# probabilists/zuko

Hardware: AMD Instinct MI355X
Metric: log_prob samples/sec, NSF d=64 K=8 bins=8 batch=2^20 (higher is better)
Workload: dtype f32; 1 GPU; NSF(features=64, context=0, transforms=8, bins=8, hidden=[256]*3) log_prob, batch=2^20 per GPU, x~N(0,1), seed-0 init; batch_per_gpu=1048576, global_batch=1048576, parallelism=batch-sharded x1, one RCCL all-reduce of the scalar NLL

## Files before the change

zuko_amd/csrc/fused_ar_half_impl.h:

```cpp
#pragma once
#include "fused_ar_split_impl.h"

#ifndef ARH_LOOK
#define ARH_LOOK 1
#endif
#ifndef ARH_RELU_INT
#define ARH_RELU_INT 0
#endif
#ifndef ARH_EPI_PINNED
#define ARH_EPI_PINNED 1
#endif
#ifndef ARH_DESCALE_PK
#define ARH_DESCALE_PK 1
#endif
#ifndef ARH_PREFETCH
#define ARH_PREFETCH 1
#endif
#ifndef ARH_BLOCK_ASM
#define ARH_BLOCK_ASM 1
#endif
#ifndef ARH_EPI_TILE
#define ARH_EPI_TILE 1
#endif

namespace zk {

typedef _Float16 f16x8 __attribute__((ext_vector_type(8)));

struct ArhB {
  f16x8 h, l;
};

__device__ __forceinline__ void arh_scale(float& amax, float& s, float& inv_s) {
  amax = fmaxf(amax, __shfl_xor(amax, 16, 64));
  amax = fmaxf(amax, __shfl_xor(amax, 32, 64));
  int e = __builtin_amdgcn_frexp_expf(amax);
  int ea = 15 - e;
  ea = ea > 90 ? 90 : (ea < -90 ? -90 : ea);
  s = __builtin_amdgcn_ldexpf(1.0f, ea);
  inv_s = __builtin_amdgcn_ldexpf(1.0f, -ea);
}

#define ARH_AMAX_OVERFLOW (65520.f * 0x1p90f)

typedef unsigned arh_u32x4 __attribute__((ext_vector_type(4)));
typedef float arh_f32x2 __attribute__((ext_vector_type(2)));

__device__ __forceinline__ void arh_split(const f32x4& lo, const f32x4& hi, float s, ArhB& b) {
  if (ARX_ABL == 6) {
    b.h = __builtin_bit_cast(f16x8, lo); b.l = __builtin_bit_cast(f16x8, hi);
    return;
  }
#if ARH_EPI_PINNED
  const float nz = -0.f;
  unsigned h0, h1, h2, h3, l0, l1, l2, l3;
#define ARH_SPLIT_H(OP, H, V) "v_fma_mix" OP "_f16 %[" H "], %[" V "], %[s], %[nz]\n\t"
#define ARH_SPLIT_L(OP, SEL, L, H, V) "v_fma_mix" OP "_f16 %[" L "], %[" V "], %[s], -%[" H "] op_sel:[0,0," SEL "] op_sel_hi:[0,0,1]\n\t"
// ... 4 lines not shown
      : [h0] "=&v"(h0), [h1] "=&v"(h1), [h2] "=&v"(h2), [h3] "=&v"(h3), [l0] "=&v"(l0), [l1] "=&v"(l1), [l2] "=&v"(l2), [l3] "=&v"(l3)
      : [v0] "v"(lo[0]), [v1] "v"(lo[1]), [v2] "v"(lo[2]), [v3] "v"(lo[3]), [v4] "v"(hi[0]), [v5] "v"(hi[1]), [v6] "v"(hi[2]), [v7] "v"(hi[3]), [s] "v"(s), [nz] "s"(nz));
#undef ARH_SPLIT_H
#undef ARH_SPLIT_L
  b.h = __builtin_bit_cast(f16x8, arh_u32x4{h0, h1, h2, h3}); b.l = __builtin_bit_cast(f16x8, arh_u32x4{l0, l1, l2, l3});
  return;
#endif
#pragma unroll
  for (int e = 0; e < 8; ++e) {
    const float v = (e < 4 ? lo[e] : hi[e - 4]) * s;
    const _Float16 h = (_Float16)v;
    const float r = v - (float)h;
    b.h[e] = h;
    b.l[e] = (_Float16)r;
  }
}

#define ARH_MFMA(A, B, C) C = __builtin_amdgcn_mfma_f32_16x16x32_f16(__builtin_bit_cast(f16x8, A), B, C, 0, 0, 0)
__device__ __forceinline__ void arh_block(const f32x4 (&a)[2], const ArhB& b, f32x4& c) {
  if (ARX_ABL == 2) {
    asm volatile("" ::"v"(a[0]), "v"(a[1]));
    return;
  }
  ARH_MFMA(a[1], b.h, c);
  ARH_MFMA(a[0], b.l, c);
  ARH_MFMA(a[0], b.h, c);
}

__device__ __forceinline__ void arh_touch(f32x4& v) { asm volatile("" : "+v"(v)); }
template <int N> __device__ __forceinline__ void arh_settle(f32x4& a0, f32x4& a1) { asm volatile("s_waitcnt lgkmcnt(%2)" : "+v"(a0), "+v"(a1) : "n"(N)); }
template <int N> __device__ __forceinline__ void arh_settle(f32x4& a0, f32x4& a1, f32x4& a2) { asm volatile("s_waitcnt lgkmcnt(%3)" : "+v"(a0), "+v"(a1), "+v"(a2) : "n"(N)); }

constexpr bool ARH_BLK = ARH_BLOCK_ASM && ARX_ABL != 2;
#define ARH_BLK_ASM(C0, COUT, POST, BSOUT)                                                                  \
  asm volatile("v_mfma_f32_16x16x32_f16 %[c], %[al], %[bh], " C0 "\n\t"                                     \
               "v_mfma_f32_16x16x32_f16 %[c], %[ah], %[bl], %[c]\n\t"                                       \
               "v_mfma_f32_16x16x32_f16 %[c], %[ah], %[bh], %[c]" POST                                      \
               : [c] COUT(c) ARH_BLK_BS##BSOUT                                                              \
               : [ah] "v"(a[0]), [al] "v"(a[1]), [bh] "v"(b.h), [bl] "v"(b.l))
#define ARH_BLK_BS0
#define ARH_BLK_BS1 , "+v"(bs)
template <int N, bool FIRST, bool PAD, bool TILE> __device__ __forceinline__ void arh_wait_block(f32x4 (&a)[2], const ArhB& b, f32x4& c, f32x4& bs) {
  static_assert(N >= 0 && N < 16, "lgkmcnt is a four-bit field");
  if constexpr (PAD) asm volatile("s_nop 0");
  __builtin_amdgcn_s_waitcnt(0xC07F | (N << 8));
  if (ARX_FENCE) __builtin_amdgcn_sched_barrier(0);
  if constexpr (FIRST && TILE) ARH_BLK_ASM("0", "=&v", "\n\ts_nop 11", 1);
  else if constexpr (FIRST) ARH_BLK_ASM("0", "=&v", "", 0);
  else if constexpr (TILE) ARH_BLK_ASM("%[c]", "+v", "\n\ts_nop 11", 1);
  else ARH_BLK_ASM("%[c]", "+v", "", 0);
  if (ARX_FENCE) __builtin_amdgcn_sched_barrier(0);
}
#undef ARH_BLK_ASM
#undef ARH_BLK_BS0
#undef ARH_BLK_BS1
template <int NT> __device__ __forceinline__ void arh_acc_ready(f32x4 (&acc)[NT]) {
  asm volatile("s_nop 11" : "+v"(acc[NT - 1]));
#pragma unroll
  for (int t = 0; t + 1 < NT; ++t) arh_touch(acc[t]);
}

__device__ __forceinline__ void arh_relu_max(f32x4& o, float (&pm)[4], int t) {
#pragma unroll
  for (int r = 0; r < 4; r += 2)
    asm("v_max_f32 %0, 0, %0\n\tv_max_f32 %1, 0, %1\n\tv_max3_f32 %2, %2, %0, %1" : "+v"(o[r]), "+v"(o[r + 1]), "+v"(pm[(2 * t + r / 2) % 4]));
}
__device__ __forceinline__ float arh_join_max(const float (&pm)[4]) {
  float amax;
  asm("v_max_f32 %0, %1, %2\n\tv_max3_f32 %0, %0, %3, %4" : "=&v"(amax) : "v"(pm[0]), "v"(pm[1]), "v"(pm[2]), "v"(pm[3]));
  return amax;
}

template <int WAVES, int CH, int NR> struct ArhRing : ArRingS<WAVES, CH, NR> {
  typedef ArRingS<WAVES, CH, NR> B;
  template <int XV> __device__ __forceinline__ void advance_x() {
    asm volatile("s_waitcnt vmcnt(%0) lgkmcnt(0)" ::"n"((NR - 2) * B::PER + XV) : "memory");
    if (ARX_ABL != 4) __builtin_amdgcn_s_barrier();
    asm volatile("" ::: "memory");
    this->issue();
    this->slot = (this->slot + 1 == NR) ? 0 : this->slot + 1;
    this->cur_off = this->lds_off + (unsigned)(this->slot * CH * AR_TF * 4 + this->lane * 16);
  }
  template <int S, int XV = 0> __device__ __forceinline__ f32x4 read() {
    if constexpr (XV != 0 && S % CH == 0) {
      advance_x<XV>();
      f32x4 v;
      if (ARX_ABL == 5) {
        asm volatile("v_mov_b32 %0, %1" : "=v"(v[0]) : "v"(this->cur_off));
// ... 73 lines not shown
      wait<XV, DRAIN>();
    }
    if (ARX_ABL != 4) __builtin_amdgcn_s_barrier();
    asm volatile("" ::: "memory");
    issue();
    asm volatile("" ::: "memory");
  }
  template <int S, int XV = 0> __device__ __forceinline__ f32x4 read() {
    static_assert(S >= 0 && S < IMAGES, "stream position");
    if constexpr (S % CH == 0) {
      read_off = (read_off + CHB == NR * CHB) ? 0 : read_off + CHB;
      cur_off = lane_off + read_off;
    }
    f32x4 v;
    if (ARX_ABL == 5) {
      asm volatile("v_mov_b32 %0, %1" : "=v"(v[0]) : "v"(cur_off));
      v[1] = v[2] = v[3] = v[0];
    } else {
      asm volatile("ds_read_b128 %0, %1 offset:%2" : "=v"(v) : "v"(cur_off), "n"((S % CH) * AR_TF * 4));
    }
    if constexpr (S == trigger(S / CH)) boundary<XV, (S % CH != BPOS + 1)>();
    if constexpr (FLOW && NCH >= 2) {
      if constexpr (S == trigger(NCH - 2)) bias_request();
    }
    return v;
  }
};

template <class S, int L, bool ALT> constexpr int arh_ip(int s) {
  if constexpr (ALT) return S::B_IP_ALT[s];
  else return ArxPat<S>::ip(L, s);
}
template <class S> constexpr bool ARH_EPI = S::ACT == 1 && ARH_EPI_PINNED && ARH_EPI_TILE;
template <class S, int L, class Ring, bool ALT = false> __device__ __forceinline__ void arh_hidden(Ring& ring, const float* bias_q, const ArhB (&in)[S::TMAX / 2], f32x4 (&out)[S::TMAX], float d, float (&pm)[4]) {
  typedef ArxPat<S> P;
  constexpr int NB = S::NB[L], BASE = S::BASE[L], HTL = S::HT[L];
  ars_for<HTL>([&](auto t_) ARS_ALWAYS_INLINE {
    constexpr int t = t_;
    if constexpr (!P::tile_has_blocks(L, t)) {
      out[t] = *reinterpret_cast<const f32x4*>(bias_q + t * 16);
      if constexpr (ARH_EPI<S>) arh_relu_max(out[t], pm, t);
    }
  });
  if constexpr (NB > 0) {
    constexpr int LOOK = ARH_LOOK < NB ? ARH_LOOK : NB;
    f32x4 a[LOOK + 1][2];
    f32x4 bs;
    f32x4 acc;
    const unsigned bias_addr = arx_lds_addr(bias_q);
    ars_for<LOOK>([&](auto b_) ARS_ALWAYS_INLINE {
      constexpr int b = b_;
      ars_for<2>([&](auto p) ARS_ALWAYS_INLINE { a[b][p] = ring.template read<BASE + 2 * b + decltype(p)::value>(); });
    });
    ars_for<NB>([&](auto s_) ARS_ALWAYS_INLINE {
      constexpr int s = s_, ot = P::ot(L, s), cur = s % (LOOK + 1);
      constexpr int ip = arh_ip<S, L, ALT>(s);
      constexpr bool first_of_tile = (s == 0 || P::ot(L, s - 1) != ot), last_of_tile = (s + 1 == NB || P::ot(L, s + 1) != ot);
      if constexpr (first_of_tile && !ARH_BLK) acc = f32x4{0.f, 0.f, 0.f, 0.f};
      if constexpr (last_of_tile) bs = arx_lds_raw<ot * 64>(bias_addr);
      if constexpr (s + LOOK < NB) {
        constexpr int nx = (s + LOOK) % (LOOK + 1);
        ars_for<2>([&](auto p) ARS_ALWAYS_INLINE { a[nx][p] = ring.template read<BASE + 2 * (s + LOOK) + decltype(p)::value>(); });
      }
      constexpr int ahead = (s + LOOK < NB ? LOOK : NB - 1 - s);
      if constexpr (ARH_BLK) {
        arh_wait_block<(last_of_tile ? (s + LOOK < NB ? 2 : 0) : 2 * ahead), first_of_tile, s == 0, last_of_tile>(a[cur], in[ip], acc, bs);
      } else {
        if constexpr (last_of_tile) arh_settle<(s + LOOK < NB ? 2 : 0)>(a[cur][0], a[cur][1], bs);
        else arh_settle<2 * ahead>(a[cur][0], a[cur][1]);
        if (ARX_FENCE) __builtin_amdgcn_sched_barrier(0);
        arh_block(a[cur], in[ip], acc);
        if (ARX_FENCE) __builtin_amdgcn_sched_barrier(0);
      }
      if constexpr (last_of_tile) {
        if (ARH_DESCALE_PK) {
#pragma unroll
          for (int r = 0; r < 4; r += 2) {
            const arh_f32x2 o = __builtin_elementwise_fma(arh_f32x2{acc[r], acc[r + 1]}, arh_f32x2{d, d}, arh_f32x2{bs[r], bs[r + 1]});
            out[ot][r] = o[0]; out[ot][r + 1] = o[1];
          }
        } else {
#pragma unroll
          for (int r = 0; r < 4; ++r) out[ot][r] = __builtin_fmaf(acc[r], d, bs[r]);
        }
        if constexpr (ARH_EPI<S>) arh_relu_max(out[ot], pm, ot);
      }
    });
  }
}

template <class S, int L, class Ring, bool HAS_ALT = false> __device__ __forceinline__ void arh_hidden_stack(Ring& ring, const float* bias_lds, int q, ArhB (&in)[S::TMAX / 2], f32x4 (&out)[S::TMAX], const float* wd,
                                                                                                         float& inv_s, float& poison, bool alt = false) {
  if constexpr (L < S::NH) {
    float pm[4] = {0.f, 0.f, 0.f, 0.f};
    if constexpr (HAS_ALT && L == 0) {
      static_assert(S::BASE[0] == 0, "B_IP_ALT lists the first layer's blocks");
      if (alt) arh_hidden<S, L, Ring, true>(ring, bias_lds + L * S::BIAS_STRIDE + 4 * q, in, out, wd[L] * inv_s, pm);
      else arh_hidden<S, L, Ring>(ring, bias_lds + L * S::BIAS_STRIDE + 4 * q, in, out, wd[L] * inv_s, pm);
    } else {
      arh_hidden<S, L, Ring>(ring, bias_lds + L * S::BIAS_STRIDE + 4 * q, in, out, wd[L] * inv_s, pm);
    }
    constexpr int HTL = S::HT[L];
    float amax = 0.f;
    if constexpr (S::ACT == 1 && ARH_EPI_PINNED) {
      if constexpr (!ARH_EPI_TILE) {
#pragma unroll
        for (int t = 0; t < HTL; ++t) arh_relu_max(out[t], pm, t);
      }
      amax = arh_join_max(pm);
    } else if constexpr (S::ACT == 1) {
#pragma unroll
      for (int t = 0; t < HTL; ++t)
#pragma unroll
        for (int r = 0; r < 4; ++r) {
          if (ARH_RELU_INT) out[t][r] = __builtin_bit_cast(float, max(__builtin_bit_cast(int, out[t][r]), 0));
          else out[t][r] = out[t][r] < 0.f ? 0.f : out[t][r];
          amax = fmaxf(amax, out[t][r]);
        }
    } else {
      ar_activate<S::ACT, HTL>(out, out);
#pragma unroll
      for (int t = 0; t < HTL; ++t)
#pragma unroll
        for (int r = 0; r < 4; ++r) amax = fmaxf(amax, fabsf(out[t][r]));
    }
    float s;
    arh_scale(amax, s, inv_s);
    if constexpr (S::ACT == 1 && ARH_EPI_PINNED) {
      if (!(amax < ARH_AMAX_OVERFLOW)) poison = __builtin_nanf("");
    }
    const f32x4 zero = {0.f, 0.f, 0.f, 0.f};
#pragma unroll
    for (int p = 0; p < (HTL + 1) / 2; ++p) arh_split(out[2 * p], 2 * p + 1 < HTL ? out[2 * p + 1] : zero, s, in[p]);
    arh_hidden_stack<S, L + 1, Ring, HAS_ALT>(ring, bias_lds, q, in, out, wd, inv_s, poison, alt);
  }
}

template <typename Uni> __device__ __forceinline__ void arh_flow_epilogue(float (&p)[4 * Uni::NT], const ArArgs& a, const int (&fid)[Uni::FPL], const float (&xin)[Uni::FPL], float poison, float* xr,
                                                                          const float* base, int D, bool term, float& lacc) {
  constexpr int FPL = Uni::FPL, TOTAL = Uni::TOTAL;
#pragma unroll
  for (int fi = 0; fi < FPL; ++fi) Uni::template poison<false>(p, fi * TOTAL, poison);
  auto ld = [&](int i) { return p[i]; };
#pragma unroll
  for (int fi = 0; fi < FPL; ++fi) {
    const int f = fid[fi];
    if (f >= 0) {
      float yv, lj;
      Uni::fwd(ld, fi * TOTAL, a, xin[fi], yv, lj);
      lacc += lj;
      if (term) {
        const float df = yv - base[f];
        lacc += __builtin_fmaf(-(df * df), base[D + f], base[2 * D + f]);
      } else {
        xr[f] = yv;
      }
    }
  }
}

template <class S, typename Uni, bool DIAG, bool TERM, bool FLOW, class Ring, class XReq, class Fids>
__device__ __forceinline__ void arh_pass(const ArArgs& a, Ring& ring, XReq& x_request, f32x4 (&xnext)[S::NIT], float* bias_lds, const Fids& fids, float* xr, const float* base, const ArLane& ln,
                                         int64_t tile, const float* wd, bool first, bool last, bool term, float& total, bool alt = false) {
  constexpr bool RING4 = S::NR == 4;
  static_assert(!FLOW || (RING4 && S::XLDS && S::DIN == S::D && !DIAG && !TERM), "flow pass: four-slot ring, rows in LDS, no context columns");
  constexpr int NT = Uni::NT, FPL = Uni::FPL, WAVES = S::WAVES;
  constexpr int NG = S::NG;
// ... 21 lines not shown
    for (int it = 0; it < S::NIT; ++it) {
      f32x4 v = {0.f, 0.f, 0.f, 0.f};
      if constexpr (FLOW) {
        if ((it + 1) * 16 <= S::DIN || it * 16 + 4 * q < S::DIN) v = *reinterpret_cast<const f32x4*>(xr + it * 16 + 4 * q);
      } else if (ARH_PREFETCH) {
        if ((it + 1) * 16 <= S::DIN || it * 16 + 4 * q < S::DIN) v = xnext[it];
      } else {
        if ((it + 1) * 16 <= S::DIN || it * 16 + 4 * q < S::DIN) v = *reinterpret_cast<const f32x4*>(xrow + it * 16 + 4 * q);
      }
      xin[it] = v;
    }
    xin[S::NIT] = f32x4{0.f, 0.f, 0.f, 0.f};
    poison = ar_poison_of<S::NIT>(xin);
    float amax = 0.f;
#pragma unroll
    for (int it = 0; it < S::NIT; ++it)
#pragma unroll
      for (int r = 0; r < 4; ++r) amax = fmaxf(amax, fabsf(xin[it][r]));
    if constexpr (XLDS && !FLOW) ar_rows_in<S::D>(xr, q, xin);
    float s;
    arh_scale(amax, s, inv_s);
    if constexpr (S::ACT == 1 && ARH_EPI_PINNED) {
      if (!(amax < ARH_AMAX_OVERFLOW)) poison = __builtin_nanf("");
    }
#pragma unroll
    for (int p = 0; p < (S::NIT + 1) / 2; ++p) arh_split(xin[2 * p], xin[2 * p + 1], s, in[p]);
  }

  float ladj_in = 0.f;
  if constexpr (!FLOW) {
    if (ARH_PREFETCH && a.ladj && a.accumulate && live && q == 0) ladj_in = a.ladj[n];
  }

  if constexpr (FLOW) arh_hidden_stack<S, 0, Ring, S::FLOW_ALT>(ring, bias_lds, q, in, out, wd, inv_s, poison, alt);
  else arh_hidden_stack<S, 0, Ring>(ring, bias_lds, q, in, out, wd, inv_s, poison);

  const float dl = wd[S::NH] * inv_s;
  float lacc = 0.f;
  constexpr int NBL = NSTEP * NT;
  constexpr int LOOKL = ARH_LOOK < NBL ? ARH_LOOK : NBL;
  f32x4 w[LOOKL + 1][2];
  constexpr int XPOS = []() constexpr {
    if constexpr (!ARH_PREFETCH) return -1;
    else if constexpr (RING4) return Ring::first_trigger_from(S::LAST_BASE);
    else return (S::LAST_BASE + S::CH - 1) / S::CH * S::CH;
  }();
  if constexpr (FLOW) {
    asm volatile("" ::: "memory");
    if (last) {
      x_request(tile + gridDim.x < a.n_tiles ? tile + gridDim.x : tile, xnext);
    } else {
#pragma unroll
      for (int it = 0; it < S::NIT; ++it) asm("" : "=v"(xnext[it]));
    }
    ring.rows_in_flight = last;
    asm volatile("" ::: "memory");
  } else if (ARH_PREFETCH) {
    asm volatile("" ::: "memory");
    x_request(tile + gridDim.x < a.n_tiles ? tile + gridDim.x : tile, xnext);
    asm volatile("" ::: "memory");
  }
#define ARH_READ_LAST(POS) ring.template read<(POS), ((POS) == XPOS ? S::NIT : 0)>()
  ars_for<LOOKL>([&](auto b_) ARS_ALWAYS_INLINE {
    constexpr int b = b_;
    ars_for<2>([&](auto p) ARS_ALWAYS_INLINE { w[b][p] = ARH_READ_LAST(S::LAST_BASE + 2 * b + decltype(p)::value); });
  });
  ars_for<NG>([&](auto g_) ARS_ALWAYS_INLINE {
    constexpr int g = g_, ST0 = S::GOFF[g], GN = S::GOFF[g + 1] - S::GOFF[g];
    int fid[FPL];
    float xin[FPL];
    fids.template fetch<XLDS>(g, xr, xrow, fid, xin);
    float bv[3 * FPL];
    if constexpr (TERM && !FLOW) fids.fetch_base(fid, base, S::D, bv);
    f32x4 acc[NT], bs[NT];
    if constexpr (GN == 0) {
      const float* bg = bias_last + (g * NT) * 16 + 4 * q;
      ars_for<NT>([&](auto t) ARS_ALWAYS_INLINE { bs[t] = *reinterpret_cast<const f32x4*>(bg + t * 16); });
    }
    if constexpr (GN == 0 || !ARH_BLK) ars_for<NT>([&](auto t) ARS_ALWAYS_INLINE { acc[t] = f32x4{0.f, 0.f, 0.f, 0.f}; });
    ars_for<GN>([&](auto i_) ARS_ALWAYS_INLINE {
      constexpr int st = ST0 + decltype(i_)::value, ip = S::G_IP[st];
      ars_for<NT>([&](auto t_) ARS_ALWAYS_INLINE {
        constexpr int t = t_, blk = st * NT + t, cur = blk % (LOOKL + 1);
        constexpr bool last_of_group = (decltype(i_)::value == GN - 1 && t == NT - 1);
        if constexpr (last_of_group) {
          ars_for<NT>([&](auto u) ARS_ALWAYS_INLINE { bs[u] = arx_lds_raw<(g * NT + decltype(u)::value) * 64>(bias_last_addr); });
        }
        if constexpr (blk + LOOKL < NBL) {
          constexpr int nx = (blk + LOOKL) % (LOOKL + 1);
          ars_for<2>([&](auto p) ARS_ALWAYS_INLINE { w[nx][p] = ARH_READ_LAST(S::LAST_BASE + 2 * (blk + LOOKL) + decltype(p)::value); });
        }
        constexpr int ahead = (blk + LOOKL < NBL ? LOOKL : NBL - 1 - blk);
        if constexpr (ARH_BLK) {
          arh_wait_block<(last_of_group ? (blk + LOOKL < NBL ? 2 : 0) : 2 * ahead), decltype(i_)::value == 0, blk == 0, false>(w[cur], in[ip], acc[t], bs[0]);
          if constexpr (last_of_group) {
#pragma unroll
            for (int u = 0; u < NT; ++u) arh_touch(bs[u]);
            arh_acc_ready<NT>(acc);
          }
        } else {
          if constexpr (last_of_group) arh_settle<(blk + LOOKL < NBL ? 2 : 0)>(w[cur][0], w[cur][1]);
          else arh_settle<2 * ahead>(w[cur][0], w[cur][1]);
          if constexpr (last_of_group) {
#pragma unroll
            for (int u = 0; u < NT; ++u) arh_touch(bs[u]);
          }
          if (ARX_FENCE) __builtin_amdgcn_sched_barrier(0);
          arh_block(w[cur], in[ip], acc[t]);
          if (ARX_FENCE) __builtin_amdgcn_sched_barrier(0);
        }
      });
    });
    float p[4 * NT];
    ars_for<NT>([&](auto t) ARS_ALWAYS_INLINE {
#pragma unroll
      for (int r = 0; r < 4; ++r) {
        p[4 * t + r] = __builtin_fmaf(acc[t][r], dl, bs[t][r]);
        if (ARH_POISON_ONE) asm("" : "+v"(p[4 * t + r]));
      }
    });
    if constexpr (FLOW) arh_flow_epilogue<Uni>(p, a, fid, xin, poison, xr, base, S::D, last && term, lacc);
    else ar_uni_epilogue<Uni, DIAG, XLDS, true, TERM>(p, a, fid, xin, poison, xr, n, live, S::D, lacc, bv);
  });
#undef ARH_READ_LAST
  if constexpr (FLOW) {
    lacc += __shfl_xor(lacc, 16, 64);
    lacc += __shfl_xor(lacc, 32, 64);
    total = first ? lacc : total + lacc;
    if (last) {
      if (live && q == 0) a.ladj[n] = total;
      if (!term) ar_rows_out<S::D>(xr, q, a.y + n * a.ldy, live);
    }
    return;
  }
  if (ARH_PREFETCH) ar_ladj_store<true>(a, lacc, n, live, q, ladj_in);
  if constexpr (XLDS && !TERM) ar_rows_out<S::D>(xr, q, a.y + n * a.ldy, live);
  if (!ARH_PREFETCH) ar_ladj_store(a, lacc, n, live, q);
}

template <class S, typename Uni, bool DIAG, bool TERM> __device__ __forceinline__ void arh_body(const ArArgs& a) {
  constexpr bool RING4 = S::NR == 4;
  typedef std::conditional_t<RING4, ArhRing4<S::WAVES, S::CH, S::IMAGES, S::BPOS>, ArhRing<S::WAVES, S::CH, S::NR>> Ring;
  static_assert(S::WAVES == 8 && (S::NR == 3 || S::NR == 4) && S::TMAX <= 16 && S::TMAX % 2 == 0 && S::OCC == 2, "two-part split kernels: widths <= 256, two wavefronts per SIMD");
  constexpr int NT = Uni::NT, FPL = Uni::FPL, WAVES = S::WAVES;
  constexpr int NG = S::NG;
  constexpr int NSTEP = S::GOFF[NG];
  static_assert(S::IMAGES == S::LAST_BASE + 2 * NSTEP * NT && (S::IMAGES + S::CH - 1) / S::CH == S::NCHUNK, "stream length");
  const ArLane ln;
  const int tid = ln.tid, lane = ln.lane, wave = ln.wave, j = ln.j, q = ln.q;

  Ring ring;
  if constexpr (RING4) {
    ring.start(ars_lds, a.stream, a.n_chunks, wave, lane);
  } else {
    ring.lds = ars_lds; ring.stream = a.stream; ring.n_chunks = a.n_chunks; ring.wave = wave; ring.lane = lane;
    ring.load_chunk = 0; ring.load_slot = 0;
#pragma unroll
// ... 151 lines not shown
```

zuko_amd/static_ar.py:

```python

from __future__ import annotations

import ctypes
import dataclasses
import fcntl
import hashlib
import json
import math
import os
import shutil
import subprocess
import sys
import threading

import numpy as np

HERE = os.path.dirname(os.path.abspath(__file__))
CSRC = os.path.join(HERE, "csrc")
ARS_DIR = os.path.join(HERE, "lib", "ars")
ARS_ABI = 10
UNI_TYPES = {0: "zk::UniAffine", 1: "zk::UniRqs8", 2: "zk::UniRqs4", 3: "zk::UniRqs16", 4: "zk::UniCircRqs8", 5: "zk::UniSos3x5", 6: "zk::UniBern17"}
SPLIT_ONLY_KINDS = {3, 5, 6}
_HEADERS = ("fused_ar_static_impl.h", "fused_ar_split_impl.h", "zk_ar_common.h", "zk_univariate.h", "zk_univariate_bwd.h", "zk_common.h", "zk_half.h")

# ... 12 lines not shown


def _jit_dir() -> str:
    d = os.environ.get("ZUKO_AMD_CACHE_DIR")
    return os.path.join(d, "ars") if d else ARS_DIR


def _dirs() -> list[str]:
    d = _jit_dir()
    return [ARS_DIR] if d == ARS_DIR else [d, ARS_DIR]


def _find(name: str) -> str | None:
    for d in _dirs():
        path = os.path.join(d, name)
        if os.path.exists(path):
            return path
    return None


_WARNED: set = set()


def _warn_once(key: str, msg: str) -> None:
    if key not in _WARNED:
        _WARNED.add(key)
        sys.stderr.write(f"[zuko_amd static_ar] {msg}\n")


def hipcc_flags() -> list:
    return ["-O3", "-std=c++17", "-fPIC", f"--offload-arch={_arch()}", "-Wno-unused-result", "-Wno-uninitialized", "-ffp-contract=off", f"-I{CSRC}"]


def _build_so(stem: str, source, meta: dict | None, verbose: bool, out_dir: str | None = None) -> str | None:
    have = _find(stem + ".so")
    if have is not None and (meta is None or os.path.exists(have[: -len(".so")] + ".json")):
        return have
    hipcc = _hipcc()
    if hipcc is None:
        _warn_once("nohipcc", f"no hipcc on this machine: the static-shape kernel {stem} cannot be compiled; this conditioner runs on the generic operand-split kernel "
                              "(same results; 1.1-1.6x the generated kernel's time; conditioners wider than 256 run layer by layer).  Build it where a ROCm compiler is installed (zuko_amd.static_ar.prebuild, or one call at the "
                              "target batch size) and ship zuko_amd/lib/ars/ or ZUKO_AMD_CACHE_DIR with the package.")
        return None
    d = out_dir or _jit_dir()
    try:
        os.makedirs(d, exist_ok=True)
        so = os.path.join(d, stem + ".so")
        with open(os.path.join(d, f".lock_{stem}"), "w") as lock:
            fcntl.flock(lock, fcntl.LOCK_EX)
            if os.path.exists(so) and (meta is None or os.path.exists(os.path.join(d, stem + ".json"))):
                return so
            src = os.path.join(d, stem + ".hip")
            with open(src, "w") as f:
                f.write(source())
            tmp = os.path.join(d, f".{stem}.so.{os.getpid()}")
            cmd = [hipcc, *hipcc_flags(), "-shared", "-no-hip-rt",
                   *os.environ.get("ZUKO_AMD_STATIC_CXXFLAGS", "").split(),
                   src, f"-L{_torch_lib_dir()}", "-l:libamdhip64.so", "-o", tmp]
            if verbose:
                print("[zuko_amd static_ar]", " ".join(cmd), flush=True)
            elif out_dir is None:
                _warn_once("jit", f"compiling a static-shape kernel for this conditioner on first use ({stem}, 10-25 s; ZUKO_AMD_JIT=0 disables, ZUKO_AMD_CACHE_DIR redirects)")
            r = subprocess.run(cmd, stdout=subprocess.PIPE, stderr=subprocess.STDOUT, text=True)
            if r.returncode != 0:
                sys.stderr.write(f"[zuko_amd static_ar] hipcc failed for {src}:\n{r.stdout[-2000:]}\n")
                try:
                    os.remove(tmp)
                except OSError:
                    pass
                return None
            os.replace(tmp, so)
            if meta is not None:
                with open(os.path.join(d, stem + ".json"), "w") as f:
                    json.dump(meta, f)
        return so
    except OSError as exc:
        _warn_once("oserror:" + d, f"cannot build kernels in {d} ({exc}); staying on the generic kernels (set ZUKO_AMD_CACHE_DIR to a writable directory)")
        return None


_HEADER_DIGEST: str | None = None


def _header_digest() -> str:
    global _HEADER_DIGEST
    if _HEADER_DIGEST is None:
        h = hashlib.sha256(str(ARS_ABI).encode())
        for name in _HEADERS:
            with open(os.path.join(CSRC, name), "rb") as f:
                h.update(f.read())
# ... 485 lines not shown
            _warn_once("load:" + so, f"cannot load {so}: {exc}")
            return None
        _LOADED[meta["so"]] = k
    return k


def _found(fam: Family, t: dict, l0: list | None):
    if fam.index is None:
        name = _identity(fam, t)[0] + ".so"
        so = _LOADED[name].so if name in _LOADED else _find(name)
        return None if so is None else ({"so": name, "dir": os.path.dirname(so)}, 0)
    idx = _INDEX if _INDEX is not None else _scan()
    for meta in idx.get(fam.index(t), []):
        if l0 is None or meta["l0"] == l0:
            return meta, 0
        if meta["alt"] is not None and meta["alt"] == l0:
            return meta, 1
    return None


def find_or_compile(fam: Family, t: dict, allow: bool, l0: list | None = None, verbose: bool = False, out_dir: str | None = None):
    with _LOCK:
        found = _found(fam, t, l0)
    if found is None and allow:
        meta = compile_unit(fam, t, None, verbose, out_dir)
        found = None if meta is None else (meta, 0)
    if found is None:
        return None
    with _LOCK:
        k = _load(found[0], fam.entry)
    return None if k is None else (k, found[1])


def _enabled() -> bool:
    return os.environ.get("ZUKO_AMD_NO_STATIC_AR", "0") != "1"


def jit_enabled() -> bool:
    return os.environ.get("ZUKO_AMD_JIT", "1") != "0" and _hipcc() is not None


def jit_min_rows() -> int:
    try:
        return int(os.environ.get("ZUKO_AMD_JIT_MIN_ROWS", str(1 << 15)))
    except ValueError:
        return 1 << 15


def _jit_allowed(rows: int | None) -> bool:
    return rows is not None and rows >= jit_min_rows() and jit_enabled()


def _jit_verbose() -> bool:
    return os.environ.get("ZUKO_AMD_JIT_VERBOSE", "0") == "1"


JIT_CUMULATIVE_FACTOR = 8


def effective_rows(holder, rows: int, count: bool = True) -> int:
    thr = jit_min_rows()
    seen = getattr(holder, "_jit_rows_seen", 0) + (max(int(rows), 0) if count else 0)
    try:
        holder._jit_rows_seen = seen
    except AttributeError:
        return rows
# ... 312 lines not shown
```

Measured before the change: 78.38 million samples/s.

## Interleave next-layer fp16 hi/lo operand splitting into MFMA issue gaps

After: 79.86 million samples/s (median of 6 runs). 1.9% higher.

```diff
diff --git a/zuko_amd/csrc/fused_ar_half_impl.h b/zuko_amd/csrc/fused_ar_half_impl.h
--- a/zuko_amd/csrc/fused_ar_half_impl.h
+++ b/zuko_amd/csrc/fused_ar_half_impl.h
@@ -23,6 +23,10 @@
 #define ARH_EPI_TILE 1
 #endif
 
+#ifndef ARH_SPLIT_GAPS
+#define ARH_SPLIT_GAPS 1
+#endif
+
 namespace zk {
 
 typedef _Float16 f16x8 __attribute__((ext_vector_type(8)));
@@ -93,28 +97,161 @@
 template <int N> __device__ __forceinline__ void arh_settle(f32x4& a0, f32x4& a1, f32x4& a2) { asm volatile("s_waitcnt lgkmcnt(%3)" : "+v"(a0), "+v"(a1), "+v"(a2) : "n"(N)); }
 
 constexpr bool ARH_BLK = ARH_BLOCK_ASM && ARX_ABL != 2;
-#define ARH_BLK_ASM(C0, COUT, POST, BSOUT)                                                                  \
-  asm volatile("v_mfma_f32_16x16x32_f16 %[c], %[al], %[bh], " C0 "\n\t"                                     \
-               "v_mfma_f32_16x16x32_f16 %[c], %[ah], %[bl], %[c]\n\t"                                       \
-               "v_mfma_f32_16x16x32_f16 %[c], %[ah], %[bh], %[c]" POST                                      \
-               : [c] COUT(c) ARH_BLK_BS##BSOUT                                                              \
-               : [ah] "v"(a[0]), [al] "v"(a[1]), [bh] "v"(b.h), [bl] "v"(b.l))
+constexpr bool ARH_GAPS = ARH_SPLIT_GAPS && ARH_BLK && ARH_EPI_PINNED && ARX_ABL != 6;
+struct ArhHL {
+  unsigned h0, h1, h2, h3, l0, l1, l2, l3;
+};
+#define ARH_GH(OP, H, V) "\n\tv_fma_mix" OP "_f16 %[" H "], %[" V "], %[s], %[nz]"
+#define ARH_GL(OP, SEL, L, H, V) "\n\tv_fma_mix" OP "_f16 %[" L "], %[" V "], %[s], -%[" H "] op_sel:[0,0," SEL "] op_sel_hi:[0,0,1]"
+#define ARH_G0 ARH_GH("lo", "h0", "v0")
+#define ARH_G1 ARH_GH("lo", "h1", "v2")
+#define ARH_G2 ARH_GH("lo", "h2", "v4")
+#define ARH_G3 ARH_GH("lo", "h3", "v6")
+#define ARH_G4 ARH_GH("hi", "h0", "v1")
+#define ARH_G5 ARH_GH("hi", "h1", "v3")
+#define ARH_G6 ARH_GH("hi", "h2", "v5")
+#define ARH_G7 ARH_GH("hi", "h3", "v7")
+#define ARH_G8 ARH_GL("lo", "0", "l0", "h0", "v0")
+#define ARH_G9 ARH_GL("lo", "0", "l1", "h1", "v2")
+#define ARH_G10 ARH_GL("lo", "0", "l2", "h2", "v4")
+#define ARH_G11 ARH_GL("lo", "0", "l3", "h3", "v6")
+#define ARH_G12 ARH_GL("hi", "1", "l0", "h0", "v1")
+#define ARH_G13 ARH_GL("hi", "1", "l1", "h1", "v3")
+#define ARH_G14 ARH_GL("hi", "1", "l2", "h2", "v5")
+#define ARH_G15 ARH_GL("hi", "1", "l3", "h3", "v7")
+#define ARH_G_OUT0
+#define ARH_G_IN0
+#define ARH_G_SC [s] "v"(s), [nz] "s"(nz)
+#define ARH_G_OUT1 , [h0] "=&v"(x.h0), [l0] "=&v"(x.l0)
+#define ARH_G_IN1 , [v0] "v"(lo[0]), [v1] "v"(lo[1]), ARH_G_SC
+#define ARH_G_OUT2 , [l0] "+v"(x.l0), [h1] "=&v"(x.h1)
+#define ARH_G_IN2 , [v1] "v"(lo[1]), [h0] "v"(x.h0), [v2] "v"(lo[2]), [v3] "v"(lo[3]), ARH_G_SC
+#define ARH_G_OUT3 , [l1] "=&v"(x.l1), [h2] "=&v"(x.h2)
+#define ARH_G_IN3 , [v2] "v"(lo[2]), [v3] "v"(lo[3]), [h1] "v"(x.h1), [v4] "v"(hi[0]), ARH_G_SC
+#define ARH_G_OUT4 , [h2] "+v"(x.h2), [l2] "=&v"(x.l2)
+#define ARH_G_IN4 , [v5] "v"(hi[1]), [v4] "v"(hi[0]), ARH_G_SC
+#define ARH_G_OUT5 , [h3] "=&v"(x.h3), [l3] "=&v"(x.l3)
+#define ARH_G_IN5 , [v6] "v"(hi[2]), [v7] "v"(hi[3]), ARH_G_SC
+#define ARH_G_OUT6 , [l3] "+v"(x.l3)
+#define ARH_G_IN6 , [v7] "v"(hi[3]), [h3] "v"(x.h3), [s] "v"(s)
+#define ARH_T_OUT2 [l0] "+v"(x.l0), [h1] "=&v"(x.h1), [l1] "=&v"(x.l1), [h2] "=&v"(x.h2), [l2] "=&v"(x.l2), [h3] "=&v"(x.h3), [l3] "=&v"(x.l3)
+#define ARH_T_IN2 [v1] "v"(lo[1]), [v2] "v"(lo[2]), [v3] "v"(lo[3]), [v4] "v"(hi[0]), [v5] "v"(hi[1]), [v6] "v"(hi[2]), [v7] "v"(hi[3]), [h0] "v"(x.h0), ARH_G_SC
+#define ARH_T_OUT3 [l1] "=&v"(x.l1), [h2] "=&v"(x.h2), [l2] "=&v"(x.l2), [h3] "=&v"(x.h3), [l3] "=&v"(x.l3)
+#define ARH_T_IN3 [v2] "v"(lo[2]), [v3] "v"(lo[3]), [v4] "v"(hi[0]), [v5] "v"(hi[1]), [v6] "v"(hi[2]), [v7] "v"(hi[3]), [h1] "v"(x.h1), ARH_G_SC
+#define ARH_T_OUT4 [h2] "+v"(x.h2), [l2] "=&v"(x.l2), [h3] "=&v"(x.h3), [l3] "=&v"(x.l3)
+#define ARH_T_IN4 [v4] "v"(hi[0]), [v5] "v"(hi[1]), [v6] "v"(hi[2]), [v7] "v"(hi[3]), ARH_G_SC
+#define ARH_T_OUT5 [h3] "=&v"(x.h3), [l3] "=&v"(x.l3)
+#define ARH_T_IN5 [v6] "v"(hi[2]), [v7] "v"(hi[3]), ARH_G_SC
+#define ARH_T_OUT6 [l3] "+v"(x.l3)
+#define ARH_T_IN6 [v7] "v"(hi[3]), [h3] "v"(x.h3), [s] "v"(s)
+#define ARH_BLK_ASM(C0, COUT, POST, BSOUT, G1, G2, G3, G)                                                   \
+  asm volatile("v_mfma_f32_16x16x32_f16 %[c], %[al], %[bh], " C0 G1 "\n\t"                                  \
+               "v_mfma_f32_16x16x32_f16 %[c], %[ah], %[bl], %[c]" G2 "\n\t"                                 \
+               "v_mfma_f32_16x16x32_f16 %[c], %[ah], %[bh], %[c]" G3 POST                                   \
+               : [c] COUT(c) ARH_BLK_BS##BSOUT ARH_G_OUT##G                                                 \
+               : [ah] "v"(a[0]), [al] "v"(a[1]), [bh] "v"(b.h), [bl] "v"(b.l) ARH_G_IN##G)
 #define ARH_BLK_BS0
 #define ARH_BLK_BS1 , "+v"(bs)
+#define ARH_BLK_FORM(G1, G2, G3, G)                                                               \
+  if constexpr (FIRST && TILE) ARH_BLK_ASM("0", "=&v", "\n\ts_nop 11", 1, G1, G2, G3, G);          \
+  else if constexpr (FIRST) ARH_BLK_ASM("0", "=&v", "", 0, G1, G2, G3, G);                         \
+  else if constexpr (TILE) ARH_BLK_ASM("%[c]", "+v", "\n\ts_nop 11", 1, G1, G2, G3, G);            \
+  else ARH_BLK_ASM("%[c]", "+v", "", 0, G1, G2, G3, G)
 template <int N, bool FIRST, bool PAD, bool TILE> __device__ __forceinline__ void arh_wait_block(f32x4 (&a)[2], const ArhB& b, f32x4& c, f32x4& bs) {
   static_assert(N >= 0 && N < 16, "lgkmcnt is a four-bit field");
   if constexpr (PAD) asm volatile("s_nop 0");
   __builtin_amdgcn_s_waitcnt(0xC07F | (N << 8));
   if (ARX_FENCE) __builtin_amdgcn_sched_barrier(0);
-  if constexpr (FIRST && TILE) ARH_BLK_ASM("0", "=&v", "\n\ts_nop 11", 1);
-  else if constexpr (FIRST) ARH_BLK_ASM("0", "=&v", "", 0);
-  else if constexpr (TILE) ARH_BLK_ASM("%[c]", "+v", "\n\ts_nop 11", 1);
-  else ARH_BLK_ASM("%[c]", "+v", "", 0);
+  ARH_BLK_FORM("", "", "", 0);
   if (ARX_FENCE) __builtin_amdgcn_sched_barrier(0);
 }
+template <int N, bool FIRST, bool PAD, bool TILE, int GF>
+__device__ __forceinline__ void arh_wait_block(f32x4 (&a)[2], const ArhB& b, f32x4& c, f32x4& bs, ArhHL& x, const f32x4& lo, const f32x4& hi, float s) {
+  static_assert(N >= 0 && N < 16 && GF >= 1 && GF <= 6, "lgkmcnt is a four-bit field; six forms");
+  const float nz = -0.f;
+  if constexpr (PAD) asm volatile("s_nop 0");
+  __builtin_amdgcn_s_waitcnt(0xC07F | (N << 8));
+  if (ARX_FENCE) __builtin_amdgcn_sched_barrier(0);
+  if constexpr (GF == 1) { ARH_BLK_FORM(ARH_G0, ARH_G4, ARH_G8, 1); }
+  else if constexpr (GF == 2) { ARH_BLK_FORM(ARH_G12, ARH_G1, ARH_G5, 2); }
+  else if constexpr (GF == 3) { ARH_BLK_FORM(ARH_G9, ARH_G13, ARH_G2, 3); }
+  else if constexpr (GF == 4) { ARH_BLK_FORM(ARH_G6, ARH_G10, ARH_G14, 4); }
+  else if constexpr (GF == 5) { ARH_BLK_FORM(ARH_G3, ARH_G7, ARH_G11, 5); }
+  else { ARH_BLK_FORM(ARH_G15, "", "", 6); }
+  if (ARX_FENCE) __builtin_amdgcn_sched_barrier(0);
+}
+template <int F> __device__ __forceinline__ void arh_split_tail(ArhHL& x, const f32x4& lo, const f32x4& hi, float s) {
+  static_assert(F >= 2 && F <= 6, "six forms");
+  const float nz = -0.f;
+#define ARH_T6 ARH_G15
+#define ARH_T5 ARH_G3 ARH_G7 ARH_G11 ARH_T6
+#define ARH_T4 ARH_G6 ARH_G10 ARH_G14 ARH_T5
+#define ARH_T3 ARH_G9 ARH_G13 ARH_G2 ARH_T4
+#define ARH_T2 ARH_G12 ARH_G1 ARH_G5 ARH_T3
+#define ARH_TAIL_ASM(T, F) asm("; the rest of a split" T : ARH_T_OUT##F : ARH_T_IN##F)
+  if constexpr (F == 2) ARH_TAIL_ASM(ARH_T2, 2);
+  else if constexpr (F == 3) ARH_TAIL_ASM(ARH_T3, 3);
+  else if constexpr (F == 4) ARH_TAIL_ASM(ARH_T4, 4);
+  else if constexpr (F == 5) ARH_TAIL_ASM(ARH_T5, 5);
+  else ARH_TAIL_ASM(ARH_T6, 6);
+#undef ARH_TAIL_ASM
+#undef ARH_T2
+#undef ARH_T3
+#undef ARH_T4
+#undef ARH_T5
+#undef ARH_T6
+}
+__device__ __forceinline__ void arh_split_done(const ArhHL& x, ArhB& b) {
+  b.h = __builtin_bit_cast(f16x8, arh_u32x4{x.h0, x.h1, x.h2, x.h3}); b.l = __builtin_bit_cast(f16x8, arh_u32x4{x.l0, x.l1, x.l2, x.l3});
+  asm volatile("" : "+v"(b.h), "+v"(b.l));
+}
+#undef ARH_BLK_FORM
 #undef ARH_BLK_ASM
 #undef ARH_BLK_BS0
 #undef ARH_BLK_BS1
+#undef ARH_G_OUT0
+#undef ARH_G_IN0
+#undef ARH_G_OUT1
+#undef ARH_G_IN1
+#undef ARH_G_OUT2
+#undef ARH_G_IN2
+#undef ARH_G_OUT3
+#undef ARH_G_IN3
+#undef ARH_G_OUT4
+#undef ARH_G_IN4
+#undef ARH_G_OUT5
+#undef ARH_G_IN5
+#undef ARH_G_OUT6
+#undef ARH_G_IN6
+#undef ARH_G_SC
+#undef ARH_T_OUT2
+#undef ARH_T_IN2
+#undef ARH_T_OUT3
+#undef ARH_T_IN3
+#undef ARH_T_OUT4
+#undef ARH_T_IN4
+#undef ARH_T_OUT5
+#undef ARH_T_IN5
+#undef ARH_T_OUT6
+#undef ARH_T_IN6
+#undef ARH_GH
+#undef ARH_GL
+#undef ARH_G0
+#undef ARH_G1
+#undef ARH_G2
+#undef ARH_G3
+#undef ARH_G4
+#undef ARH_G5
+#undef ARH_G6
+#undef ARH_G7
+#undef ARH_G8
+#undef ARH_G9
+#undef ARH_G10
+#undef ARH_G11
+#undef ARH_G12
+#undef ARH_G13
+#undef ARH_G14
+#undef ARH_G15
 template <int NT> __device__ __forceinline__ void arh_acc_ready(f32x4 (&acc)[NT]) {
   asm volatile("s_nop 11" : "+v"(acc[NT - 1]));
 #pragma unroll
@@ -254,9 +391,102 @@
   else return ArxPat<S>::ip(L, s);
 }
 template <class S> constexpr bool ARH_EPI = S::ACT == 1 && ARH_EPI_PINNED && ARH_EPI_TILE;
-template <class S, int L, class Ring, bool ALT = false> __device__ __forceinline__ void arh_hidden(Ring& ring, const float* bias_q, const ArhB (&in)[S::TMAX / 2], f32x4 (&out)[S::TMAX], float d, float (&pm)[4]) {
+
+template <int NBLK> struct ArhGapPlan {
+  signed char pair[NBLK > 0 ? NBLK : 1], form[NBLK > 0 ? NBLK : 1];
+  short lim[9];
+  signed char front[9];
+};
+template <class S, int L, int NT> constexpr int arh_gap_blocks() {
+  if constexpr (L == S::NH) return S::GOFF[S::NG] * NT;
+  else return S::NB[L];
+}
+template <class S, int L, int NT> constexpr int arh_gap_reader(int b) {
+  if constexpr (L == S::NH) return S::G_IP[b / NT];
+  else return ArxPat<S>::ip(L, b);
+}
+template <class S, int L> constexpr int arh_gap_last_block(int t) {
+  if (t >= S::HT[L]) return S::NB[L];
+  int last = -1;
+  for (int b = 0; b < S::NB[L]; ++b)
+    if (ArxPat<S>::ot(L, b) == t) last = b;
+  return last;
+}
+template <class S, int L, int NT> constexpr ArhGapPlan<arh_gap_blocks<S, L, NT>()> arh_gap_plan() {
+  static_assert(L >= 1 && L <= S::NH && S::TMAX / 2 <= 8, "a consuming layer; eight in pairs at most");
+  constexpr int NBLK = arh_gap_blocks<S, L, NT>(), NP = (S::HT[L - 1] + 1) / 2;
+  ArhGapPlan<NBLK> g{};
+  for (int p = 0; p < 9; ++p) { g.lim[p] = 0; g.front[p] = 7; }
+  int cursor = 0;
+  for (int p = 1; p < NP; ++p) {
+    int lim = NBLK;
+    for (int b = NBLK - 1; b >= 0; --b)
+      if (arh_gap_reader<S, L, NT>(b) == p) lim = b;
+    if constexpr (L != S::NH) {
+      for (int t = 2 * p; t <= 2 * p + 1; ++t) {
+        const int last = arh_gap_last_block<S, L>(t);
+        lim = last < 0 ? 0 : (last < lim ? last : lim);
+      }
+    }
+    int f = 1;
+    for (; f <= 6 && cursor < lim; ++f, ++cursor) { g.pair[cursor] = (signed char)p; g.form[cursor] = (signed char)f; }
+    g.lim[p] = (short)lim;
+    g.front[p] = (signed char)f;
+  }
+  return g;
+}
+template <class S, int L, int NT, bool ON> struct ArhGapsOf {
+  static constexpr int NP = 0, NBLK = 0;
+  static constexpr int form(int) { return 0; }
+  static constexpr int pair(int) { return 0; }
+  static constexpr bool tail_at(int, int) { return false; }
+  static constexpr bool any_tail_at(int) { return false; }
+  static constexpr int front(int) { return 7; }
+};
+template <class S, int L, int NT> struct ArhGapsOf<S, L, NT, true> {
+  static constexpr int NP = (S::HT[L - 1] + 1) / 2, NBLK = arh_gap_blocks<S, L, NT>();
+  static constexpr ArhGapPlan<NBLK> plan = arh_gap_plan<S, L, NT>();
+  static constexpr int form(int b) { return plan.form[b]; }
+  static constexpr int pair(int b) { return plan.pair[b]; }
+  static constexpr bool tail_at(int p, int b) { return p >= 1 && plan.front[p] <= 6 && plan.lim[p] == b; }
+  static constexpr int front(int p) { return plan.front[p]; }
+  static constexpr bool any_tail_at(int b) {
+    for (int p = 1; p < NP; ++p)
+      if (tail_at(p, b)) return true;
+    return false;
+  }
+};
+template <class GP, int HTI, int NPR> __device__ __forceinline__ void arh_gap_front(const f32x4 (&out)[2 * NPR], float s, ArhB (&in)[NPR]) {
+  const f32x4 zero = {0.f, 0.f, 0.f, 0.f};
+  arh_split(out[0], 1 < HTI ? out[1] : zero, s, in[0]);
+  ars_for<GP::NP>([&](auto p_) ARS_ALWAYS_INLINE {
+    constexpr int p = p_;
+    if constexpr (GP::tail_at(p, 0)) arh_split(out[2 * p], 2 * p + 1 < HTI ? out[2 * p + 1] : zero, s, in[p]);
+  });
+}
+template <class GP, int HTI, int B, int NPR> __device__ __forceinline__ void arh_gap_tails(ArhHL (&x)[NPR], const f32x4 (&out)[2 * NPR], float s, ArhB (&in)[NPR]) {
+  const f32x4 zero = {0.f, 0.f, 0.f, 0.f};
+  ars_for<GP::NP>([&](auto p_) ARS_ALWAYS_INLINE {
+    constexpr int p = p_;
+    if constexpr (B >= 1 && GP::tail_at(p, B)) {
+      if constexpr (GP::front(p) == 1) {
+        arh_split(out[2 * p], 2 * p + 1 < HTI ? out[2 * p + 1] : zero, s, in[p]);
+      } else {
+        arh_split_tail<GP::front(p)>(x[p], out[2 * p], 2 * p + 1 < HTI ? out[2 * p + 1] : zero, s);
+        arh_split_done(x[p], in[p]);
+      }
+    }
+  });
+}
+
+template <class S, int L, class Ring, bool ALT = false, bool GAPS = false>
+__device__ __forceinline__ void arh_hidden(Ring& ring, const float* bias_q, ArhB (&in)[S::TMAX / 2], f32x4 (&out)[S::TMAX], float d, float (&pm)[4], float s_in = 0.f) {
   typedef ArxPat<S> P;
-  constexpr int NB = S::NB[L], BASE = S::BASE[L], HTL = S::HT[L];
+  typedef ArhGapsOf<S, L, 0, GAPS> GP;
+  constexpr int NB = S::NB[L], BASE = S::BASE[L], HTL = S::HT[L], HTI = S::HT[L > 0 ? L - 1 : 0];
+  ArhHL x[S::TMAX / 2];
+  const f32x4 zero = {0.f, 0.f, 0.f, 0.f};
+  if constexpr (GAPS) arh_gap_front<GP, HTI>(out, s_in, in);
   ars_for<HTL>([&](auto t_) ARS_ALWAYS_INLINE {
     constexpr int t = t_;
     if constexpr (!P::tile_has_blocks(L, t)) {
@@ -285,8 +515,15 @@
         ars_for<2>([&](auto p) ARS_ALWAYS_INLINE { a[nx][p] = ring.template read<BASE + 2 * (s + LOOK) + decltype(p)::value>(); });
       }
       constexpr int ahead = (s + LOOK < NB ? LOOK : NB - 1 - s);
-      if constexpr (ARH_BLK) {
-        arh_wait_block<(last_of_tile ? (s + LOOK < NB ? 2 : 0) : 2 * ahead), first_of_tile, s == 0, last_of_tile>(a[cur], in[ip], acc, bs);
+      if constexpr (GAPS) arh_gap_tails<GP, HTI, s>(x, out, s_in, in);
+      constexpr int WAIT = last_of_tile ? (s + LOOK < NB ? 2 : 0) : 2 * ahead;
+      constexpr bool pad = s == 0 || (GAPS && s >= 1 && GP::any_tail_at(s));
+      if constexpr (GP::form(s) != 0) {
+        constexpr int gp = GP::pair(s);
+        arh_wait_block<WAIT, first_of_tile, pad, last_of_tile, GP::form(s)>(a[cur], in[ip], acc, bs, x[gp], out[2 * gp], 2 * gp + 1 < HTI ? out[2 * gp + 1] : zero, s_in);
+        if constexpr (GP::form(s) == 6) arh_split_done(x[gp], in[gp]);
+      } else if constexpr (ARH_BLK) {
+        arh_wait_block<WAIT, first_of_tile, pad, last_of_tile>(a[cur], in[ip], acc, bs);
       } else {
         if constexpr (last_of_tile) arh_settle<(s + LOOK < NB ? 2 : 0)>(a[cur][0], a[cur][1], bs);
         else arh_settle<2 * ahead>(a[cur][0], a[cur][1]);
@@ -308,11 +545,12 @@
         if constexpr (ARH_EPI<S>) arh_relu_max(out[ot], pm, ot);
       }
     });
+    if constexpr (GAPS) arh_gap_tails<GP, HTI, NB>(x, out, s_in, in);
   }
 }
 
 template <class S, int L, class Ring, bool HAS_ALT = false> __device__ __forceinline__ void arh_hidden_stack(Ring& ring, const float* bias_lds, int q, ArhB (&in)[S::TMAX / 2], f32x4 (&out)[S::TMAX], const float* wd,
-                                                                                                         float& inv_s, float& poison, bool alt = false) {
+                                                                                                         float& inv_s, float& poison, float& s, bool alt = false) {
   if constexpr (L < S::NH) {
     float pm[4] = {0.f, 0.f, 0.f, 0.f};
     if constexpr (HAS_ALT && L == 0) {
@@ -320,7 +558,7 @@
       if (alt) arh_hidden<S, L, Ring, true>(ring, bias_lds + L * S::BIAS_STRIDE + 4 * q, in, out, wd[L] * inv_s, pm);
       else arh_hidden<S, L, Ring>(ring, bias_lds + L * S::BIAS_STRIDE + 4 * q, in, out, wd[L] * inv_s, pm);
     } else {
-      arh_hidden<S, L, Ring>(ring, bias_lds + L * S::BIAS_STRIDE + 4 * q, in, out, wd[L] * inv_s, pm);
+      arh_hidden<S, L, Ring, false, ARH_GAPS && L >= 1>(ring, bias_lds + L * S::BIAS_STRIDE + 4 * q, in, out, wd[L] * inv_s, pm, s);
     }
     constexpr int HTL = S::HT[L];
     float amax = 0.f;
@@ -346,15 +584,16 @@
 #pragma unroll
         for (int r = 0; r < 4; ++r) amax = fmaxf(amax, fabsf(out[t][r]));
     }
-    float s;
     arh_scale(amax, s, inv_s);
     if constexpr (S::ACT == 1 && ARH_EPI_PINNED) {
       if (!(amax < ARH_AMAX_OVERFLOW)) poison = __builtin_nanf("");
     }
-    const f32x4 zero = {0.f, 0.f, 0.f, 0.f};
-#pragma unroll
-    for (int p = 0; p < (HTL + 1) / 2; ++p) arh_split(out[2 * p], 2 * p + 1 < HTL ? out[2 * p + 1] : zero, s, in[p]);
-    arh_hidden_stack<S, L + 1, Ring, HAS_ALT>(ring, bias_lds, q, in, out, wd, inv_s, poison, alt);
+    if constexpr (!ARH_GAPS) {
+      const f32x4 zero = {0.f, 0.f, 0.f, 0.f};
+#pragma unroll
+      for (int p = 0; p < (HTL + 1) / 2; ++p) arh_split(out[2 * p], 2 * p + 1 < HTL ? out[2 * p + 1] : zero, s, in[p]);
+    }
+    arh_hidden_stack<S, L + 1, Ring, HAS_ALT>(ring, bias_lds, q, in, out, wd, inv_s, poison, s, alt);
   }
 }
 
@@ -442,8 +681,14 @@
     if (ARH_PREFETCH && a.ladj && a.accumulate && live && q == 0) ladj_in = a.ladj[n];
   }
 
-  if constexpr (FLOW) arh_hidden_stack<S, 0, Ring, S::FLOW_ALT>(ring, bias_lds, q, in, out, wd, inv_s, poison, alt);
-  else arh_hidden_stack<S, 0, Ring>(ring, bias_lds, q, in, out, wd, inv_s, poison);
+  float s_last = 0.f;
+  if constexpr (FLOW) arh_hidden_stack<S, 0, Ring, S::FLOW_ALT>(ring, bias_lds, q, in, out, wd, inv_s, poison, s_last, alt);
+  else arh_hidden_stack<S, 0, Ring>(ring, bias_lds, q, in, out, wd, inv_s, poison, s_last);
+  typedef ArhGapsOf<S, S::NH, Uni::NT, (ARH_GAPS && S::NH >= 1)> GP;
+  constexpr int HTI = S::HT[S::NH >= 1 ? S::NH - 1 : 0];
+  ArhHL hl[S::TMAX / 2];
+  const f32x4 zero = {0.f, 0.f, 0.f, 0.f};
+  if constexpr (ARH_GAPS && S::NH >= 1) arh_gap_front<GP, HTI>(out, s_last, in);
 
   const float dl = wd[S::NH] * inv_s;
   float lacc = 0.f;
@@ -501,8 +746,17 @@
           ars_for<2>([&](auto p) ARS_ALWAYS_INLINE { w[nx][p] = ARH_READ_LAST(S::LAST_BASE + 2 * (blk + LOOKL) + decltype(p)::value); });
         }
         constexpr int ahead = (blk + LOOKL < NBL ? LOOKL : NBL - 1 - blk);
+        if constexpr (ARH_GAPS && S::NH >= 1) arh_gap_tails<GP, HTI, blk>(hl, out, s_last, in);
+        constexpr int WAIT = last_of_group ? (blk + LOOKL < NBL ? 2 : 0) : 2 * ahead;
+        constexpr bool pad = blk == 0 || (ARH_GAPS && S::NH >= 1 && blk >= 1 && GP::any_tail_at(blk));
         if constexpr (ARH_BLK) {
-          arh_wait_block<(last_of_group ? (blk + LOOKL < NBL ? 2 : 0) : 2 * ahead), decltype(i_)::value == 0, blk == 0, false>(w[cur], in[ip], acc[t], bs[0]);
+          if constexpr (GP::form(blk) != 0) {
+            constexpr int gp = GP::pair(blk);
+            arh_wait_block<WAIT, decltype(i_)::value == 0, pad, false, GP::form(blk)>(w[cur], in[ip], acc[t], bs[0], hl[gp], out[2 * gp], 2 * gp + 1 < HTI ? out[2 * gp + 1] : zero, s_last);
+            if constexpr (GP::form(blk) == 6) arh_split_done(hl[gp], in[gp]);
+          } else {
+            arh_wait_block<WAIT, decltype(i_)::value == 0, pad, false>(w[cur], in[ip], acc[t], bs[0]);
+          }
           if constexpr (last_of_group) {
 #pragma unroll
             for (int u = 0; u < NT; ++u) arh_touch(bs[u]);
@@ -533,6 +787,7 @@
     else ar_uni_epilogue<Uni, DIAG, XLDS, true, TERM>(p, a, fid, xin, poison, xr, n, live, S::D, lacc, bv);
   });
 #undef ARH_READ_LAST
+  if constexpr (ARH_GAPS && S::NH >= 1) arh_gap_tails<GP, HTI, NBL>(hl, out, s_last, in);
   if constexpr (FLOW) {
     lacc += __shfl_xor(lacc, 16, 64);
     lacc += __shfl_xor(lacc, 32, 64);
diff --git a/zuko_amd/static_ar.py b/zuko_amd/static_ar.py
--- a/zuko_amd/static_ar.py
+++ b/zuko_amd/static_ar.py
@@ -68,8 +68,8 @@
     return ["-O3", "-std=c++17", "-fPIC", f"--offload-arch={_arch()}", "-Wno-unused-result", "-Wno-uninitialized", "-ffp-contract=off", f"-I{CSRC}"]
 
 
-def _build_so(stem: str, source, meta: dict | None, verbose: bool, out_dir: str | None = None) -> str | None:
-    have = _find(stem + ".so")
+def _build_so(stem: str, source, meta: dict | None, verbose: bool, out_dir: str | None = None, only_dir: bool = False, cxxflags: list | None = None) -> str | None:
+    have = (os.path.join(out_dir, stem + ".so") if os.path.exists(os.path.join(out_dir, stem + ".so")) else None) if only_dir else _find(stem + ".so")
     if have is not None and (meta is None or os.path.exists(have[: -len(".so")] + ".json")):
         return have
     hipcc = _hipcc()
@@ -91,7 +91,7 @@
                 f.write(source())
             tmp = os.path.join(d, f".{stem}.so.{os.getpid()}")
             cmd = [hipcc, *hipcc_flags(), "-shared", "-no-hip-rt",
-                   *os.environ.get("ZUKO_AMD_STATIC_CXXFLAGS", "").split(),
+                   *(os.environ.get("ZUKO_AMD_STATIC_CXXFLAGS", "").split() if cxxflags is None else cxxflags),
                    src, f"-L{_torch_lib_dir()}", "-l:libamdhip64.so", "-o", tmp]
             if verbose:
                 print("[zuko_amd static_ar]", " ".join(cmd), flush=True)
@@ -643,6 +643,46 @@
     return None if k is None else (k, found[1])
 
 
+def build_half_variant(configs: list, out_dir: str, cxxflags: list | None = None, jobs: int = 4) -> list:
+    from concurrent.futures import ThreadPoolExecutor
+
+    ars = os.path.join(os.path.abspath(out_dir), "ars")
+    work = []
+    for cfg in configs:
+        tabs = [half_tables(plan, layout.kind, 1) for plan, layout, _ in _plans_for(*cfg)]
+        if any(t is None for t in tabs):
+            raise ValueError(f"no two-part kernel for {cfg}")
+        for t, _ in tabs:
+            if (ARH, t) not in work:
+                work.append((ARH, t))
+        tf = flow_tables([t for t, _ in tabs])
+        if tf is not None:
+            work.append((ARHF, tf[0]))
+
+    def one(w):
+        fam, t = w
+        stem, meta = _identity(fam, t)
+        return _build_so(stem, lambda: emit(fam, t), dict(meta, flags=list(cxxflags or [])), False, ars, only_dir=True, cxxflags=list(cxxflags or []))
+
+    with ThreadPoolExecutor(max_workers=jobs) as ex:
+        sos = list(ex.map(one, work))
+    if any(so is None for so in sos):
+        raise RuntimeError("zuko_amd.static_ar: a variant kernel failed to compile")
+    rescan()
+    return sos
+
+
+def rescan() -> None:
+    global _INDEX
+    with _LOCK:
+        _INDEX = None
+
+
+def loaded_kernels() -> dict:
+    with _LOCK:
+        return {name: k.so for name, k in _LOADED.items()}
+
+
 def _enabled() -> bool:
     return os.environ.get("ZUKO_AMD_NO_STATIC_AR", "0") != "1"
 
```
